# nicholasburden/pymarl

Hardware: AMD Instinct MI355X
Metric: learner samples/sec (B×T×n_agents), synthetic replay, 1/2/4/8 MI355X (higher is better)
Workload: dtype fp32; 1 GPU; QMIX synthetic replay n_agents=8 T=120 obs=80 state=168 batch=32; mixer=qmix, n_agents=8, n_actions=14, obs_dim=80, state_dim=168, episode_limit=120, batch_per_gpu=32, global_batch=32, replay_episodes=5000, parallelism=dp1

## Files before the change

include/mq_learner.h:

```cpp
#ifndef MQ_LEARNER_H
#define MQ_LEARNER_H

#include <stdint.h>

#ifdef __cplusplus
extern "C" {
#endif

enum { MQ_MIXER_NONE = 0, MQ_MIXER_VDN = 1, MQ_MIXER_QMIX = 2 };
enum { MQ_OK = 0, MQ_ERR_ARG = 1, MQ_ERR_HIP = 2, MQ_ERR_STATE = 3 };
enum { MQ_NSUMS = 8 };
enum { MQ_NSTATS = 8 };

enum {
  MQ_P_FC1_W, MQ_P_FC1_B, MQ_P_RNN_W_IH, MQ_P_RNN_W_HH, MQ_P_RNN_B_IH, MQ_P_RNN_B_HH, MQ_P_FC2_W, MQ_P_FC2_B,
  MQ_P_HW1_W, MQ_P_HW1_B, MQ_P_HWF_W, MQ_P_HWF_B, MQ_P_HB1_W, MQ_P_HB1_B, MQ_P_V0_W, MQ_P_V0_B, MQ_P_V2_W,
  MQ_P_V2_B, MQ_P_COUNT
};

typedef struct mq_config {
  int32_t n_agents, n_actions, obs_dim, state_dim;
  int32_t rnn_hidden_dim;
  int32_t mixing_embed_dim;
  int32_t mixer;
// ... 52 lines not shown
                   float* q_out, int32_t which, void* stream);
int mq_agent_forward(mq_handle* h, const float* inputs, int32_t rows, const float* h_in, float* h_out,
                     float* q_out, int32_t which, void* stream);
int mq_greedy_actions(const float* q, const int32_t* avail, int64_t* out, int32_t rows, int32_t n_actions,
                      void* stream);

int mq_qmix_forward(const float* mixer, int32_t n_agents, int32_t state_dim, int32_t embed_dim,
                    const float* agent_qs, const float* states, float* q_tot, int32_t rows, void* stream);

enum { MQ_HYP_NONE = 0, MQ_HYP_WS = 1, MQ_HYP_LDS = 2, MQ_HYP_GEMM = 3 };
enum { MQ_MIX_FAST16 = 0, MQ_MIX_FAST32 = 1, MQ_MIX_GENERIC = 2, MQ_MIX_STREAM = 3 };
typedef struct mq_plan {
  int32_t rows;
  int32_t fused_fwd;
  int32_t rw_fwd;
  int32_t fused_bwd;
  int32_t rw_bwd;
  int32_t inline_ids;
  int32_t hyper;
  int32_t mix;
  int32_t tiles;
  int32_t dwh;
  int32_t td_lambda;
} mq_plan;
int mq_last_plan(const mq_handle* h, mq_plan* out);

int mq_set_timing(mq_handle* h, int32_t slots, uint32_t phase_mask);
int mq_phase_times(mq_handle* h, float* ms, int32_t cap, int32_t* n);
const char* mq_phase_names(void);

#ifdef __cplusplus
}
#endif
#endif
```

pymarl_amd/_lib.py:

```python
from __future__ import annotations

import ctypes
import os

HERE = os.path.dirname(os.path.abspath(__file__))
LIB_PATH = os.environ.get("MQ_LEARNER_LIB", os.path.join(HERE, "lib", "libmq_learner.so"))

MIXER_NONE, MIXER_VDN, MIXER_QMIX = 0, 1, 2
NSUMS = 8
NSTATS = 8
PARAM_NAMES = [
    "fc1.weight", "fc1.bias", "rnn.weight_ih", "rnn.weight_hh", "rnn.bias_ih", "rnn.bias_hh", "fc2.weight",
    "fc2.bias", "hyper_w_1.weight", "hyper_w_1.bias", "hyper_w_final.weight", "hyper_w_final.bias",
    "hyper_b_1.weight", "hyper_b_1.bias", "V.0.weight", "V.0.bias", "V.2.weight", "V.2.bias",
]
P_COUNT = len(PARAM_NAMES)

EXPORTS = [
    "mq_last_error", "mq_create", "mq_destroy", "mq_param_offsets", "mq_bind", "mq_forward_backward", "mq_apply",
    "mq_train_step", "mq_update_targets", "mq_copy_intermediate", "mq_mac_forward", "mq_agent_forward",
    "mq_greedy_actions", "mq_set_timing", "mq_phase_times", "mq_phase_names", "mq_set_data_parallel",
    "mq_last_plan", "mq_qmix_forward",
    "mc_create", "mc_destroy", "mc_param_offsets", "mc_bind", "mc_train_step", "mc_update_targets", "mc_policy",
    "mc_copy_intermediate", "mc_set_timing", "mc_phase_times", "mc_last_critic_path", "mq_comm_unique_id", "mq_comm_attach",
# ... 26 lines not shown
class MQReplay(ctypes.Structure):
    _fields_ = [
        ("obs", ctypes.c_void_p), ("state", ctypes.c_void_p), ("actions", ctypes.c_void_p),
        ("avail_actions", ctypes.c_void_p), ("reward", ctypes.c_void_p), ("terminated", ctypes.c_void_p),
        ("filled", ctypes.c_void_p), ("ep_ids", ctypes.c_void_p), ("n_episodes", ctypes.c_int64),
        ("batch_size", ctypes.c_int32), ("t_len", ctypes.c_int32), ("t_stride", ctypes.c_int32),
        ("ep_ids_host", ctypes.c_void_p), ("avail_bits", ctypes.c_void_p),
    ]


class MCConfig(ctypes.Structure):
    _fields_ = [
        ("n_agents", ctypes.c_int32), ("n_actions", ctypes.c_int32), ("obs_dim", ctypes.c_int32),
        ("state_dim", ctypes.c_int32), ("rnn_hidden_dim", ctypes.c_int32), ("obs_last_action", ctypes.c_int32),
        ("obs_agent_id", ctypes.c_int32), ("mask_before_softmax", ctypes.c_int32), ("gamma", ctypes.c_float),
        ("td_lambda", ctypes.c_float), ("lr", ctypes.c_float), ("critic_lr", ctypes.c_float),
        ("optim_alpha", ctypes.c_float), ("optim_eps", ctypes.c_float), ("grad_norm_clip", ctypes.c_float),
        ("max_batch", ctypes.c_int32), ("max_seq", ctypes.c_int32),
    ]


class MQPlan(ctypes.Structure):
    _fields_ = [(k, ctypes.c_int32) for k in ("rows", "fused_fwd", "rw_fwd", "fused_bwd", "rw_bwd", "inline_ids",
                                               "hyper", "mix", "tiles", "dwh", "td_lambda")]

    def as_dict(self):
        return {k: int(getattr(self, k)) for k, _ in self._fields_}


HYP_NAMES = {0: "none", 1: "ws", 2: "lds", 3: "gemm"}
MIX_NAMES = {0: "fast16", 1: "fast32", 2: "generic", 3: "stream"}

INLINE_IDS = 256
COMM_ID_BYTES = 128


_LIB = None


class MQError(RuntimeError):
    pass


def load(required=True):
    global _LIB
    if _LIB is not None:
        return _LIB
# ... 134 lines not shown
```

pymarl_amd/csrc/gru_bwd_fused.hpp:

```cpp
#pragma once
#include <cstdlib>
#include "gru_fwd_fused.hpp"
#include "dwh_kernel.hpp"

namespace mq {

constexpr int BRP = 4 * H + 4;

struct alignas(16) BwdFusedLds {
  float gh[2][FCH][BRP];
  float gi[2][FCH][BRP];
  float x1[FCH][H + 4];
  float xin[FCH][FXP];
  float dx1[FCH][H + 4];
  float db1[4][H];
  float wih[G3][H + 1];
};

inline bool fused_bwd_ok(int I, int O, int A, int n, int64_t RT) { return fused_fwd_ok(I, O, A, n, RT); }

constexpr int BSTH = 16, BSTN = BSTH + 152;
template <int DWH = 0, bool STAMP = false>
__global__ __launch_bounds__(512) void gru_bwd_fused_kernel(Dims d, Rep rp, const float* __restrict__ P, Lay L,
                                                            Work w, int64_t slab_len, int64_t slab1_len) {
  __shared__ BwdFusedLds S;
  extern __shared__ float dyn[];
  __shared__ uint32_t bst[STAMP ? BSTN : 1];
  auto bstamp = [&](int slot) {
    if constexpr (STAMP) {
      uint64_t tt;
      __builtin_amdgcn_sched_barrier(0);
      asm volatile("s_memtime %0\n\ts_waitcnt lgkmcnt(0)" : "=s"(tt)::"memory");
      __builtin_amdgcn_sched_barrier(0);
      if ((threadIdx.x & 63) == 0) bst[slot] = (uint32_t)tt;
    }
  };
  if (threadIdx.x == 0) bstamp(0);
  if constexpr (DWH != 0) {
    static_assert(sizeof(BwdFusedLds) >= 2 * 4 * DWH_T * (DWH_T + 1) * sizeof(float), "dW_hyper tiles reuse the LDS");
    if ((int)blockIdx.x >= d.R) {
      const int half = (int)threadIdx.x >> 8;
      const int lin = min(2 * ((int)blockIdx.x - d.R) + half, w.dwh_n - 1);
      dwh_body<8, 4>(d, L, w.dHYP, w.S0, w.slab_mix, w.dwh_len, w.dwh_ns, w.dwh_tj, lin, (int)threadIdx.x & 255,
                        (float*)&S + half * 4 * DWH_T * (DWH_T + 1));
      return;
// ... 43 lines not shown
    const int b3 = (c16 >> 3) & 1, b2 = (c16 >> 2) & 1, u0 = 4 * (lt >> 4);
    f32x4 xr[12];
    {
      const float* Whh = P + L.o[MQ_P_RNN_W_HH];
#pragma unroll
      for (int kk = 0; kk < 12; ++kk) xr[kk] = *(const f32x4*)(Whh + (12 * c16 + kk) * H + u0);
    }
    auto k12_sum = [&](const f32x4 (&dv)[3]) {
      f32x2 aA = {0.0f, 0.0f}, aB = {0.0f, 0.0f};
#pragma unroll
      for (int m = 0; m < 3; ++m)
#pragma unroll
        for (int e = 0; e < 4; ++e) {
          const f32x2 dd = {dv[m][e], dv[m][e]};
          aA = pk_fma(wT[2 * (4 * m + e)], dd, aA);
          aB = pk_fma(wT[2 * (4 * m + e) + 1], dd, aB);
        }
      const float x = aA.x + row_ror8(aB.x), y = aA.y + row_ror8(aB.y);
      return quad_sum(x + row_half_mirror(y));
    };
    struct In { float g, aux, w2, wd, ci, ch, hq, gz; };
    const float* aux_base;
    int64_t aux_stride;
    if (q == 0) { aux_base = w.Hs + (int64_t)r * H + k - (int64_t)R * H; aux_stride = (int64_t)R * H; }
    else if (q == 3) { aux_base = (const float*)arow; aux_stride = 2 * (int64_t)d.n; }
    else { aux_base = w.dch + r; aux_stride = R; }
    const float* g_base = w.Gates + (int64_t)r * (4 * H) + q * H + k;
    const int e0 = q == 0 ? 1 : 0, e12 = (q == 1 || q == 2) ? 1 : 0;
    auto load = [&](int t, In& s) {
      const int tc = max(t, 0);
      const int idx = tc + (e0 & (tc == 0 ? 1 : 0)) - (e12 & (tc >= T ? 1 : 0));
      s.g = g_base[(int64_t)tc * R * (4 * H)];
      s.aux = aux_base[idx * aux_stride];
    };
    auto lookup_w2 = [&](In& s) { s.w2 = w2_s[__builtin_bit_cast(int, quad_bcast<3>(s.aux)) * H + k]; };
    const float m0 = q == 0 ? 1.0f : 0.0f, m1 = q == 1 ? 1.0f : 0.0f, m2 = q == 2 ? 1.0f : 0.0f;
    const float m3 = q == 3 ? 1.0f : 0.0f;
    float carry = 0.0f, db_i = 0.0f, db_h = 0.0f;
    auto coeffs = [&](int t, In& s) {
      const float gr = quad_bcast<0>(s.g), gz = quad_bcast<1>(s.g), gn = quad_bcast<2>(s.g), ghn = quad_bcast<3>(s.g);
      const float hp = t > 0 ? quad_bcast<0>(s.aux) : 0.0f;
      const float dchv = t < T ? quad_bcast<2>(s.aux) : 0.0f;
      const float an = (1.0f - gz) * (1.0f - gn * gn);
      const float ar = (an * ghn) * (gr * (1.0f - gr));
      const float az = (hp - gn) * (gz * (1.0f - gz));
      const float rzc = fmaf(m0, ar, m1 * az);
      s.ci = fmaf(m2 + m3, an, rzc);
      s.ch = fmaf(m2, an * gr, rzc);
      s.hq = m3 * hp;
      s.wd = dchv * s.w2;
      s.gz = gz;
    };
    auto lstep = [&](int t, const In& cur, In& nxt, In& ahead) {
      load(t - 3, ahead);
      const int p = t & (FCH - 1), cb = (t / FCH) & 1;
      const float dh = carry + cur.wd;
      const float mine_i = dh * cur.ci;
      const float mine_h = fmaf(dh, cur.ch, cur.hq);
      S.gh[cb][p][q * H + k] = mine_h;
      S.gi[cb][p][q * H + k] = mine_i;
      db_i = fmaf(1.0f - m3, mine_i, db_i);
      db_h = fmaf(1.0f - m3, mine_h, db_h);
      lds_barrier();
      const f32x4* d12 = (const f32x4*)(&S.gh[cb][p][12 * c16]);
      const f32x4 dv[3] = {d12[0], d12[1], d12[2]};
      lookup_w2(nxt);
      coeffs(t - 1, nxt);
      carry = fmaf(dh, cur.gz, k12_sum(dv));
      if constexpr (STAMP) { if (tid < 64 && Tp - 1 - t < BSTN - BSTH) bstamp(BSTH + Tp - 1 - t); }
    };
    In sa, sb, sc, sd;
    load(Tp - 1, sa);
    load(Tp - 2, sb);
    load(Tp - 3, sc);
    stage_common();
    {
      const int a0 = u0 + 2 * b3 + b2, a1 = u0 + 2 * b3 + 1 - b2;
      const int v0 = u0 + 2 * (1 - b3) + b2, v1 = u0 + 2 * (1 - b3) + 1 - b2;
      auto pick = [](const f32x4& x, int i) { return i == 0 ? x[0] : i == 1 ? x[1] : i == 2 ? x[2] : x[3]; };
      const int i0 = a0 - u0, i1 = a1 - u0, i2 = v0 - u0, i3 = v1 - u0;
#pragma unroll
      for (int kk = 0; kk < 12; ++kk) {
        wT[2 * kk] = f32x2{pick(xr[kk], i0), pick(xr[kk], i1)};
        wT[2 * kk + 1] = f32x2{pick(xr[kk], i2), pick(xr[kk], i3)};
      }
    }
    drain_vmem();
    lds_barrier();
    if (tid == 0) bstamp(1);
    lookup_w2(sa);
    coeffs(Tp - 1, sa);
    int t = Tp - 1;
    for (; t - 3 >= 0; t -= 4) {
      lstep(t, sa, sb, sd);
      lstep(t - 1, sb, sc, sa);
      lstep(t - 2, sc, sd, sb);
      lstep(t - 3, sd, sa, sc);
    }
    if (t >= 0) lstep(t, sa, sb, sd);
    if (t - 1 >= 0) lstep(t - 1, sb, sc, sa);
    if (t - 2 >= 0) lstep(t - 2, sc, sd, sb);
    if (tid == 0) bstamp(2);
    lds_barrier();
    lds_barrier();
    if (q < 3) { slab[o_bi + q * H + k] = db_i; slab[o_bh + q * H + k] = db_h; }
  } else {
    const int ptid = tid - 256, wv = ptid >> 6, lane = ptid & 63, g = lane >> 4, c16 = lane & 15;
    const int Kq = (I + 15) / 16 * 4;
    f32x4 acc_hh[3][4], acc_ih[3][4], acc_w1[7];
#pragma unroll
    for (int i = 0; i < 3; ++i)
#pragma unroll
      for (int jj = 0; jj < 4; ++jj) { acc_hh[i][jj] = f32x4{0, 0, 0, 0}; acc_ih[i][jj] = f32x4{0, 0, 0, 0}; }
#pragma unroll
    for (int i = 0; i < 7; ++i) acc_w1[i] = f32x4{0, 0, 0, 0};
    f32x4 dxa = {0, 0, 0, 0}, dxb = {0, 0, 0, 0};
    float db1p = 0.0f;

    constexpr int NX1 = FCH * H / 256, NXI = (FCH * 4 * FKQ + 255) / 256;
    float rx1[NX1], rxi[NXI];
    auto issue_rows = [&](int C) {
      const int t0 = FCH * C;
#pragma unroll
      for (int s = 0; s < NX1; ++s) {
// ... 72 lines not shown
          if (16 * nt >= 4 * Kq) break;
          acc_w1[nt] = mfma16x4(av, S.xin[row][16 * nt + c16], acc_w1[nt]);
        }
      }
    };
    float h_next = 0.0f, dch_n = 0.0f;
    int act_n = 0;
    auto fc2_fetch = [&](int t) {
      const int tc = max(t, 0);
      dch_n = w.dch[(int64_t)min(tc, T - 1) * R + r];
      act_n = *(const int*)(arow + (int64_t)tc * d.n);
    };
    auto fc2_grads = [&](int t) {
      const int p = t & (FCH - 1), cb = (t / FCH) & 1;
      const float dchv = t < T ? dch_n : 0.0f;
      const int a = act_n;
      fc2_fetch(t - 1);
      if (t < T && (a & 3) == q) {
        dw2_s[a * H + k] += dchv * h_next;
        if (k == 0) db2_s[a] += dchv;
      }
      h_next = S.gh[cb][p][3 * H + k];
    };
    fc2_fetch(Tp - 1);
    issue_rows(cl);
    stage_common();

    lds_barrier();
    for (int c = cl; c >= 0; --c) {
      const int C = c + 1;
      const bool work = C <= cl;
#pragma unroll
      for (int u = 0; u < FCH; ++u) {
        const int t = FCH * c + FCH - 1 - u;
        if (t >= Tp) continue;
        lds_barrier();
        fc2_grads(t);
        if (work) {
          if (u >= 1 && u <= 4) dw_rec(C, u - 1, u, false);
          if (u == 4) store_rows(C);
          if (u >= 5 && u <= 8) dw_rec(C, u - 5, u - 4, true);
          if (u >= 9 && u <= 12) dx1_part(C, 3 * (u - 9), 3 * (u - 8));
          if (u == 12) dx1_epi();
          if (u == 13) dw1_part(0, 1);
          if (u == 14) dw1_part(1, 2);
          if (u == 15) dw1_part(2, 4);
        }
        if (u == 5 && c < cl) issue_rows(c);
      }
    }
    auto write_rec = [&](const f32x4 (&acc)[3][4], int64_t o) {
#pragma unroll
      for (int i = 0; i < 3; ++i)
#pragma unroll
        for (int jj = 0; jj < 4; ++jj)
          *(f32x4*)&slab[o + (((3 * wv + i) * 4 + jj) * 64 + lane) * 4] = acc[i][jj];
    };
    dw_rec(0, 0, 4, false);
    if (ptid == 0) bstamp(6);
    store_rows(0);
    write_rec(acc_hh, o_hh);
    if (ptid == 0) bstamp(7);
    lds_barrier();
    if (ptid == 0) bstamp(8);
    dw_rec(0, 0, 4, true);
    if (ptid == 0) bstamp(9);
    write_rec(acc_ih, 0);
    if (ptid == 0) bstamp(10);
    dx1_part(0, 0, 12);
    dx1_epi();
    if (ptid == 0) bstamp(11);
    lds_barrier();
    dw1_part(0, 4);
    if (ptid == 0) bstamp(3);

    float* slab1 = w.slab_fc1 + (int64_t)blockIdx.x * slab1_len;
#pragma unroll
    for (int nt = 0; nt < 7; ++nt)
#pragma unroll
      for (int e = 0; e < 4; ++e) {
        const int m = 16 * wv + 4 * g + e, nn = 16 * nt + c16;
        if (nn < I) slab1[m * I + nn] = acc_w1[nt][e];
      }
    S.db1[g][16 * wv + c16] = db1p;
  }
  lds_barrier();
  if (tid == 0) bstamp(4);
  for (int i = tid; i < A * H; i += 512) slab[o_w2 + i] = dw2_s[i];
  for (int i = tid; i < A; i += 512) slab[o_b2 + i] = db2_s[i];
  if (tid < H)
    w.slab_fc1[(int64_t)blockIdx.x * slab1_len + H * I + tid] =
        (S.db1[0][tid] + S.db1[1][tid]) + (S.db1[2][tid] + S.db1[3][tid]);
  if constexpr (STAMP) {
    asm volatile("s_waitcnt vmcnt(0)" ::: "memory");
    __syncthreads();
    if (tid == 0) bstamp(5);
    __syncthreads();
    if (blockIdx.x < 8)
      for (int i = tid; i < BSTN; i += 512) ((uint32_t*)w.GI)[(size_t)blockIdx.x * BSTN + i] = bst[i];
  }
}

inline void launch_bwd_fused_dwh(size_t dyn, hipStream_t s, const Dims& d, const Rep& rp, const float* P,
                                 const Lay& L, const Work& w, int64_t slab_len, int64_t slab1_len) {
  const dim3 grid(d.R + (w.dwh_n + 1) / 2);
  hipLaunchKernelGGL((gru_bwd_fused_kernel<1>), grid, dim3(512), dyn, s, d, rp, P, L, w, slab_len, slab1_len);
}
inline void launch_bwd_fused(dim3 grid, size_t dyn, hipStream_t s, const Dims& d, const Rep& rp, const float* P,
                             const Lay& L, const Work& w, int64_t slab_len, int64_t slab1_len, bool stamp = false) {
  if (stamp)
    hipLaunchKernelGGL((gru_bwd_fused_kernel<0, true>), grid, dim3(512), dyn, s, d, rp, P, L, w, slab_len, slab1_len);
  else
    hipLaunchKernelGGL((gru_bwd_fused_kernel<0>), grid, dim3(512), dyn, s, d, rp, P, L, w, slab_len, slab1_len);
}

}
```

pymarl_amd/csrc/gru_fwd_pair.hpp:

```cpp
#pragma once
#include "gru_fwd_fused.hpp"

namespace mq {

struct alignas(16) PairLds {
  float h0[H];
  int psync[4];
  float xin[2][FCH][FXP];
  float x1[2][2][FCH][H + 4];
  float hs[2][2][FCH][H + 4];
  float gi[2][2][FCH][G3];
  f32x4 grec[2][FCH][H];
};
static_assert(sizeof(PairLds) - offsetof(PairLds, hs) >= 2 * G3 * H * sizeof(float), "W_hh staging fits");
constexpr int kPairPrologueBarriers = 3;

inline bool pair_fwd_ok(int I, int O, int A, int n, int64_t RT) { return fused_fwd_ok(I, O, A, n, RT); }

constexpr int PSH = 32;
constexpr int PST = PSH + 2 * 512;
MQ_DEV uint32_t stamp_now() {
  uint64_t t;
  __builtin_amdgcn_sched_barrier(0);
  asm volatile("s_memtime %0\n\ts_waitcnt lgkmcnt(0)" : "=s"(t)::"memory");
// ... 379 lines not shown
      for (int e = 0; e < 4; ++e) S.gi[z][cc & 1][4 * g + e][16 * (3 * pw + s) + c16] = accg[s][e] + bih[z][s];
  };
  auto fc2 = [&](int cc) {
    const int z = pw;
    f32x4 q0 = {0, 0, 0, 0}, q1 = {0, 0, 0, 0};
#pragma unroll
    for (int kq = 0; kq < 4; ++kq) {
      const f32x4 av = *(const f32x4*)&S.hs[z][cc & 1][c16][16 * g + 4 * kq];
      q0 = mfma16x4(av[0], w2r[4 * kq], q0);
      q1 = mfma16x4(av[1], w2r[4 * kq + 1], q1);
      q0 = mfma16x4(av[2], w2r[4 * kq + 2], q0);
      q1 = mfma16x4(av[3], w2r[4 * kq + 3], q1);
    }
    const int t0 = FCH * cc;
    const auto qb = buf_rsrc(w.Q + (int64_t)z * d.RT() * A + ((int64_t)t0 * R + r) * A);
    const uint32_t lo = (uint32_t)(4 * g) * RA + c16;
#pragma unroll
    for (int e = 0; e < 4; ++e)
      buf_st(qb, (t0 + 4 * g + e < Tp && c16 < A) ? (lo + e * RA) * 4 : kDrop, (q0[e] + q1[e]) + b2);
  };

  auto store_records = [&](int cc) {
    const int t0 = FCH * cc, j = ptid & 63;
#pragma unroll
    for (int k = 0; k < 4; ++k) {
      const int i = 4 * k + (ptid >> 6), t = t0 + i;
      const f32x4 gv = S.grec[cc & 1][i][j];
      const float hv = S.hs[0][cc & 1][i][j];
      const bool ok = t < Tp;
      buf_st(buf_rsrc(w.Hs + (int64_t)min(t, Tp - 1) * RH), ok ? ((uint32_t)r * H + j) * 4 : kDrop, hv);
      const auto gb = buf_rsrc(w.Gates + (int64_t)min(t, Tp - 1) * (4 * RH));
      const uint32_t go = ((uint32_t)r * (4 * H) + j) * 4;
#pragma unroll
      for (int q = 0; q < 4; ++q) buf_st(gb, ok ? go + q * 4 * H : kDrop, gv[q]);
    }
  };

  if (pw == 0) stamp(16);
  store_gather(0);
  if (cl >= 1) issue_gather(1);
  if (pw == 0) stamp(17);
  lds_barrier();
  if (pw == 0) stamp(18);
  fc1(0, 0);
  fc1(1, 0);
  if (cl >= 1) { store_gather(1); if (cl >= 2) issue_gather(2); }
// ... 90 lines not shown
```

pymarl_amd/csrc/learner_types.hpp:

```cpp
#pragma once
#include "common.hpp"
#include "../../include/mq_learner.h"

namespace mq {

constexpr int H = 64;
constexpr int G3 = 3 * H;

struct Dims {
  int n, A, O, S, E, I, NH;
  int B, Tp, T, R, M;
  int t_stride;
  int last_action, agent_id, mixer, double_q;
  float gamma;
  float huber;
  FastDiv dR, dN, dB, dO, dI, dS;
  MQ_DEV int64_t RT() const { return (int64_t)Tp * R; }
};

MQ_DEV float td_loss(float mtd, float delta) {
  if (delta > 0.0f) {
    const float ax = fabsf(mtd);
    return ax <= delta ? 0.5f * mtd * mtd : delta * (ax - 0.5f * delta);
  }
// ... 26 lines not shown
  float* X1;
  float* GI;
  float* Hs;
  float* Gates;
  float* Q;
  float* HYP;
  float* dHYP;
  float* dch;
  float* dGI;
  float* dP1;
  float* slab_fc1;
  float* slab_rnn;
  float* slab_mix;
  float* slab_v2;
  float* loss_part;
  float* norm_part;
  int32_t* curmax;
  float* red_tmp;
  float* XIN;
  float* S0;
  float* dHo;
  int64_t dwh_len = 0;
  int dwh_ns = 0, dwh_tj = 0, dwh_n = 0;
};

MQ_DEV void split_tr(const Dims& d, uint32_t tr, int& t, int& r, int& b, int& ag) {
  t = (int)fdiv(tr, d.dR);
  r = (int)tr - t * d.R;
  b = (int)fdiv((uint32_t)r, d.dN);
  ag = r - b * d.n;
}

}
```

pymarl_amd/csrc/mq_learner.hip:

```cpp
#include <cstdio>
#include <cstdlib>
#include <algorithm>
#include <cstring>
#include <mutex>
#include <string>
#include <vector>

#include <rccl/rccl.h>
#include "learner_gemms.hpp"
#include "gru_kernels.hpp"
#include "gru_fwd_fused.hpp"
#include "gru_fwd_pair.hpp"
#include "gru_bwd_fused.hpp"
#include "gru_tiles.hpp"
#include "mix_kernels.hpp"
#include "td_lambda_kernel.hpp"
#include "hyper_kernel.hpp"
#include "dwh_kernel.hpp"
#include "optim_kernels.hpp"
#include "module_fwd.hpp"
#include "switches.hpp"

using namespace mq;

// ... 76 lines not shown
  float *on = nullptr, *tg = nullptr, *grad = nullptr, *sq = nullptr, *stats = nullptr;
  int32_t* curmax_user = nullptr;
  void* ws = nullptr;
  Work w;
  int32_t* curmax_ws = nullptr;
  bool have_fb = false;
  Dims last;
  mq_plan plan{};
  int nsplit_fc1 = 1, nsplit_mix = 1, nblk_bwd = 1, nblk_mix = 1, n_norm_part = 0;
  bool force_unfused = plan_flag("unfused_fwd");
  bool force_unfused_bwd = plan_flag("unfused_bwd");
  static constexpr int fused_bwd_rmax = 512;
  int dwh_split = plan_int("dwh_split", 8);
  int row_tiles = plan_int("row_tiles", -1);
  bool dp = false;
  ncclComm_t comm = nullptr;
  int comm_world = 0;
  bool comm_owned = false;
  hipStream_t side = nullptr;
  hipEvent_t ev_fork = nullptr, ev_join = nullptr;
  int hyp_in_fwd = plan_int("hyp_in_fwd", -1);
  int dwh_in_bwd = plan_int("dwh_in_bwd", -1);
  int fwd_pair = plan_int("fwd_pair", -1);
  bool pair_hyp_epi = plan_flag("pair_hyp_epi");
  bool mix_generic = plan_flag("mix_generic");
  bool lambda_path = plan_int("lambda_path", 0) != 0;
  float *YT = nullptr, *G = nullptr;
  bool have_lambda = false;
  int num_cu = 0;
  int slots = 0;
  uint32_t mask = 0;
  int64_t tstep = 0;
  std::vector<hipEvent_t> ev0, ev1;
  std::vector<uint8_t> ev_used;
};

namespace {

void compute_layout(mq_handle* h) {
  const mq_config& c = h->cfg;
  const int Hd = mq::H, n = c.n_agents, A = c.n_actions, S = c.state_dim, E = h->E, I = h->I;
  int64_t sz[MQ_P_COUNT] = {};
  sz[MQ_P_FC1_W] = (int64_t)Hd * I; sz[MQ_P_FC1_B] = Hd;
  sz[MQ_P_RNN_W_IH] = 3LL * Hd * Hd; sz[MQ_P_RNN_W_HH] = 3LL * Hd * Hd;
  sz[MQ_P_RNN_B_IH] = 3 * Hd; sz[MQ_P_RNN_B_HH] = 3 * Hd;
  sz[MQ_P_FC2_W] = (int64_t)A * Hd; sz[MQ_P_FC2_B] = A;
// ... 225 lines not shown
  mq_handle* h = new mq_handle();
  h->cfg = c;
  h->E = c.mixer == MQ_MIXER_QMIX ? c.mixing_embed_dim : 0;
  h->I = c.obs_dim + (c.obs_last_action ? c.n_actions : 0) + (c.obs_agent_id ? c.n_agents : 0);
  h->NH = h->E * (c.n_agents + 3);
  compute_layout(h);

  const int64_t n = c.n_agents, A = c.n_actions, Hd = mq::H;
  const int64_t RT = (int64_t)c.max_seq * c.max_batch * n;
  const int64_t Mm = (int64_t)(c.max_seq - 1) * c.max_batch;
  const int64_t Rm = (int64_t)c.max_batch * n;
  const int64_t nmix = (Mm + 3) / 4;
  const int64_t NH = h->NH;
  auto ng = [](int64_t ns) { return std::min<int64_t>(ns, kRedZ); };
  const int64_t nfc1 = std::max<int64_t>(kNsplitMax, Rm);
  const int64_t red_tmp = ng(Rm) * h->len_rnn + ng(nfc1) * (Hd * h->I + Hd) + ng(kNsplitMax) * h->len_mix +
                          ng(nmix) * (h->E + 1) + ng(nmix) * 8;
  const int64_t norm_parts = (Hd * h->I + Hd + 255) / 256 + (h->len_rnn + 255) / 256 + (h->len_mix + 255) / 256 +
                             (h->E + 1 + 255) / 256 + 1 + 8;
  int64_t sizes[20] = {
      2 * RT * Hd,
      2 * RT * 3 * Hd,
      2 * RT * Hd,
      RT * 4 * Hd,
      2 * RT * A,
      2 * Mm * NH,
      Mm * NH,
      Mm * n,
      RT * 3 * Hd,
      RT * Hd,
      nfc1 * (Hd * h->I + Hd),
      Rm * h->pitch_rnn,
      (int64_t)kNsplitMax * h->len_mix,
      nmix * (h->E + 1),
      nmix * 8,
      std::max<int64_t>(norm_parts, 256),
      Mm * n,
      red_tmp,
      RT * h->I,
      Mm * c.state_dim,
  };
  int64_t total = 0, offs[20];
  for (int i = 0; i < 20; ++i) { offs[i] = total; total += align_up(std::max<int64_t>(sizes[i], 1)); }
  hipError_t e = hipMalloc(&h->ws, total * sizeof(float));
  if (e != hipSuccess) {
    delete h;
    return set_err(MQ_ERR_HIP, std::string("workspace hipMalloc(") + std::to_string(total * 4) + " B): " +
// ... 71 lines not shown
    return set_err(MQ_ERR_STATE, "training needs online, target, grad, sq_avg and stats bound (mq_bind)");
  int rc = check_batch(h, batch);
  if (rc) return rc;
  const Dims d = make_dims(h, batch);
  const Rep rp = make_rep(batch);
  const Lay L = make_lay(h);
  Work w = h->w;
  int32_t* curmax = h->curmax_user ? h->curmax_user : h->curmax_ws;
  const int64_t RT = (int64_t)d.Tp * d.R;
  PhaseTimer pt{h, s};
  const mq_config& c = h->cfg;

  mq_plan plan{};
  plan.rows = d.R;
  plan.inline_ids = rp.nids > 0 ? 1 : 0;
  const int rw_bwd = std::min(2, pick_rw(d.R, 256));
  const int kq1 = tile_kq1(d.O);
  const bool tiles = tiles_ok(d.I, d.O, d.A, d.n, d.Tp, RT) && !h->force_unfused && !h->force_unfused_bwd &&
                     (h->row_tiles == 1 || (h->row_tiles < 0 && d.R > 512));
  const bool fused_bwd = !tiles && d.R <= h->fused_bwd_rmax && fused_bwd_ok(d.I, d.O, d.A, d.n, RT) &&
                         !h->force_unfused_bwd;
  const int rw_fwd = pick_rw(d.R, 512);
  bool hyp_in_fwd = false;
  plan.tiles = tiles ? 1 : 0;
  if (tiles) {
    pt.begin(PH_GRUF);
    const dim3 grid(16 * (((d.R + TR_F - 1) / TR_F + 7) / 8));
    const float *P0 = h->on, *P1 = h->tg;
    if (kq1 == 8) hipLaunchKernelGGL(gru_fwd_tile_kernel<8>, grid, dim3(512), 0, s, d, rp, P0, P1, L, w);
    else if (kq1 == 20) hipLaunchKernelGGL(gru_fwd_tile_kernel<20>, grid, dim3(512), 0, s, d, rp, P0, P1, L, w);
    else if (kq1 == 40) hipLaunchKernelGGL(gru_fwd_tile_kernel<40>, grid, dim3(512), 0, s, d, rp, P0, P1, L, w);
    else if (kq1 == 72) hipLaunchKernelGGL(gru_fwd_tile_kernel<72>, grid, dim3(512), 0, s, d, rp, P0, P1, L, w);
    else hipLaunchKernelGGL(gru_fwd_tile_kernel<80>, grid, dim3(512), 0, s, d, rp, P0, P1, L, w);
    MQ_HIP(hipGetLastError());
  } else if (rw_fwd == 1 && fused_fwd_ok(d.I, d.O, d.A, d.n, RT) && !h->force_unfused) {
    plan.fused_fwd = 1;
    pt.begin(PH_GRUF);
    const bool two_waves = device_cus(h) > 0 && d.R > h->num_cu;
    const bool pair = h->hyp_in_fwd != 1 && pair_fwd_ok(d.I, d.O, d.A, d.n, RT) &&
                      (h->fwd_pair == 1 || (h->fwd_pair < 0 && !two_waves && device_cus(h) > 0));
    hyp_in_fwd = !pair && (h->hyp_in_fwd == 1 || (h->hyp_in_fwd < 0 && two_waves)) && c.mixer == MQ_MIXER_QMIX &&
                 hyper_ws_ok(d.S, d.E, d.NH, d.M) && hyf_ok(d.S, d.E, d.NH, d.M);
    if (hyp_in_fwd) {
      plan.hyper = MQ_HYP_WS;
      launch_fwd_fused_hyp(s, d, rp, (const float*)h->on, (const float*)h->tg, L, w);
    } else if (pair) {
      plan.fused_fwd = 2;
      hyp_in_fwd = h->hyp_in_fwd != 0 && c.mixer == MQ_MIXER_QMIX && hyper_ws_ok(d.S, d.E, d.NH, d.M) &&
                   hyf_ok(d.S, d.E, d.NH, d.M);
      if (hyp_in_fwd) plan.hyper = MQ_HYP_WS;
      std::string stamp_path;
      const bool want_stamp = env_item("MQ_DIAG", "pair_stamp", &stamp_path) && !stamp_path.empty();
      const int hsched = env_int("MQ_DIAG", "hyp_sched", kHypSched, 16);
      const int pair_hyp = !hyp_in_fwd ? 0 : (2 * ((d.M + 31) / 32) <= d.R && !h->pair_hyp_epi) ? 2 : 1;
      const bool stamp = want_stamp && d.Tp <= 512 && FCH * d.O <= 256 * 5;
      launch_fwd_pair(s, d, rp, (const float*)h->on, (const float*)h->tg, L, w, pair_hyp, stamp, hsched);
      if (stamp) {
        std::vector<uint32_t> st((size_t)8 * PST);
        MQ_HIP(hipMemcpyAsync(st.data(), w.slab_rnn, st.size() * 4, hipMemcpyDeviceToHost, s));
        MQ_HIP(hipStreamSynchronize(s));
        if (FILE* f = fopen(stamp_path.c_str(), "ab")) { fwrite(st.data(), 4, st.size(), f); fclose(f); }
      }
    } else {
      launch_fwd_fused(dim3(d.R, 2), s, d, rp, (const float*)h->on, (const float*)h->tg, L, w);
    }
    MQ_HIP(hipGetLastError());
  } else {
    plan.rw_fwd = rw_fwd;
    pt.begin(PH_FC1);
    {
      Fc1Prob p{d, rp, h->on, h->tg, h->off[MQ_P_FC1_W], h->off[MQ_P_FC1_B], w.X1, w.XIN, RT};
      MQ_HIP(launch_gemm(p, (int)RT, 2 * mq::H, 1, s));
    }
    pt.begin(PH_GI);
    {
      GiProb p{w.X1, h->on, h->tg, h->off[MQ_P_RNN_W_IH], h->off[MQ_P_RNN_B_IH], w.GI, RT};
      MQ_HIP(launch_gemm(p, (int)RT, mq::G3, 2, s));
    }
// ... 83 lines not shown
  } else if (fused_bwd) {
    const bool many = device_cus(h) > 0 && d.R > h->num_cu;
    h->nblk_bwd = d.R;
    h->nsplit_fc1 = h->nblk_bwd;
    const size_t dyn = ((size_t)2 * d.A * mq::H + d.A) * sizeof(float);
    if (c.mixer == MQ_MIXER_QMIX) {
      const int tj = (d.NH + DWH_T - 1) / DWH_T, ts = (d.S + 1 + DWH_T - 1) / DWH_T;
      dwh_mode = h->dwh_in_bwd >= 0 ? (h->dwh_in_bwd ? 1 : 0) : many ? 1 : 0;
      if (dwh_mode != 0) {
        w.dwh_tj = tj;
        w.dwh_ns = dwh_ns;
        w.dwh_n = tj * ts * dwh_ns;
        w.dwh_len = h->len_mix;
        h->nsplit_mix = dwh_ns;
      }
    }
    dwh_in_bwd = dwh_mode != 0;
    plan.dwh = dwh_mode;
    const float* P0 = (const float*)h->on;
    const int64_t l1 = (int64_t)mq::H * d.I + mq::H;
    std::string bstamp_path;
    const bool bstamp = dwh_mode != 1 && env_item("MQ_DIAG", "bwd_stamp", &bstamp_path) && !bstamp_path.empty() &&
                        d.Tp <= BSTN - BSTH;
    if (dwh_mode == 1) MQ_LDS(gru_bwd_fused_kernel<1>, dyn);
    else MQ_LDS((gru_bwd_fused_kernel<0, true>), dyn);
    if (dwh_mode == 1) launch_bwd_fused_dwh(dyn, s, d, rp, P0, L, w, h->pitch_rnn, l1);
    else launch_bwd_fused(dim3(d.R), dyn, s, d, rp, P0, L, w, h->pitch_rnn, l1, bstamp);
    if (bstamp) {
      std::vector<uint32_t> st((size_t)8 * BSTN);
      MQ_HIP(hipMemcpyAsync(st.data(), w.GI, st.size() * 4, hipMemcpyDeviceToHost, s));
      MQ_HIP(hipStreamSynchronize(s));
      if (FILE* f = fopen(bstamp_path.c_str(), "ab")) { fwrite(st.data(), 4, st.size(), f); fclose(f); }
    }
    MQ_HIP(hipGetLastError());
  } else {
    {
      const size_t dyn = ((size_t)2 * d.A * mq::H + d.A) * sizeof(float);
      if (rw_bwd == 1) MQ_LDS(gru_bwd_kernel<1>, dyn);
      else if (rw_bwd == 2) MQ_LDS(gru_bwd_kernel<2>, dyn);
      else MQ_LDS(gru_bwd_kernel<4>, dyn);
      hipError_t e = rw_bwd == 1 ? launch_gru_bwd<1>(d, rp, h, L, w, s, &h->nblk_bwd)
                   : rw_bwd == 2 ? launch_gru_bwd<2>(d, rp, h, L, w, s, &h->nblk_bwd)
                                 : launch_gru_bwd<4>(d, rp, h, L, w, s, &h->nblk_bwd);
      MQ_HIP(e);
    }
    pt.begin(PH_DX1);
    {
      Dx1Prob p{w.dGI, h->on + h->off[MQ_P_RNN_W_IH], w.X1, w.dP1, RT};
      MQ_HIP(launch_gemm(p, (int)RT, mq::H, 1, s));
    }
// ... 304 lines not shown
```

Before: 154.7 million samples/s.

## Add lean fused GRU backward with precomputed gate coefficients and walked addressing

Adds a lean variant of the fused GRU backward kernel, on by default when the paired forward path runs. The forward pair kernel now stores precomputed GRU derivative coefficients (ar, az, an, anr, gz) into a widened 5H gate record. The backward loads these instead of recomputing them on its serial time recurrence, and walks pointers for addressing instead of computing per-step indices. The fc2 gradient accumulation becomes register-resident packed FMAs fed from lane-broadcast prefetches. In exchange the Gates buffer grows by a quarter, and the forward does extra stores and arithmetic.

```diff
diff --git a/include/mq_learner.h b/include/mq_learner.h
--- a/include/mq_learner.h
+++ b/include/mq_learner.h
@@ -98,6 +98,7 @@
   int32_t tiles;
   int32_t dwh;
   int32_t td_lambda;
+  int32_t bwd_lean;
 } mq_plan;
 int mq_last_plan(const mq_handle* h, mq_plan* out);
 
diff --git a/pymarl_amd/_lib.py b/pymarl_amd/_lib.py
--- a/pymarl_amd/_lib.py
+++ b/pymarl_amd/_lib.py
@@ -72,7 +72,7 @@
 
 class MQPlan(ctypes.Structure):
     _fields_ = [(k, ctypes.c_int32) for k in ("rows", "fused_fwd", "rw_fwd", "fused_bwd", "rw_bwd", "inline_ids",
-                                               "hyper", "mix", "tiles", "dwh", "td_lambda")]
+                                               "hyper", "mix", "tiles", "dwh", "td_lambda", "bwd_lean")]
 
     def as_dict(self):
         return {k: int(getattr(self, k)) for k, _ in self._fields_}
diff --git a/pymarl_amd/csrc/gru_bwd_fused.hpp b/pymarl_amd/csrc/gru_bwd_fused.hpp
--- a/pymarl_amd/csrc/gru_bwd_fused.hpp
+++ b/pymarl_amd/csrc/gru_bwd_fused.hpp
@@ -1,5 +1,6 @@
 #pragma once
 #include <cstdlib>
+#include <type_traits>
 #include "gru_fwd_fused.hpp"
 #include "dwh_kernel.hpp"
 
@@ -19,8 +20,10 @@
 
 inline bool fused_bwd_ok(int I, int O, int A, int n, int64_t RT) { return fused_fwd_ok(I, O, A, n, RT); }
 
+constexpr int LEAN_ADDR = 1, LEAN_FC2 = 2, LEAN_COEF = 4;
+constexpr int kBwdLean = LEAN_ADDR | LEAN_FC2 | LEAN_COEF;
 constexpr int BSTH = 16, BSTN = BSTH + 152;
-template <int DWH = 0, bool STAMP = false>
+template <int DWH = 0, bool STAMP = false, int LEAN = 0>
 __global__ __launch_bounds__(512) void gru_bwd_fused_kernel(Dims d, Rep rp, const float* __restrict__ P, Lay L,
                                                             Work w, int64_t slab_len, int64_t slab1_len) {
   __shared__ BwdFusedLds S;
@@ -110,37 +113,56 @@
     struct In { float g, aux, w2, wd, ci, ch, hq, gz; };
     const float* aux_base;
     int64_t aux_stride;
+    constexpr bool COEF = (LEAN & LEAN_COEF) != 0;
+    constexpr int GP = COEF ? 5 * H : 4 * H;
     if (q == 0) { aux_base = w.Hs + (int64_t)r * H + k - (int64_t)R * H; aux_stride = (int64_t)R * H; }
     else if (q == 3) { aux_base = (const float*)arow; aux_stride = 2 * (int64_t)d.n; }
+    else if (COEF && q == 1) { aux_base = w.Gates + (int64_t)r * GP + 4 * H + k; aux_stride = (int64_t)R * GP; }
     else { aux_base = w.dch + r; aux_stride = R; }
-    const float* g_base = w.Gates + (int64_t)r * (4 * H) + q * H + k;
-    const int e0 = q == 0 ? 1 : 0, e12 = (q == 1 || q == 2) ? 1 : 0;
+    const float* g_base = w.Gates + (int64_t)r * GP + q * H + k;
+    const int e0 = q == 0 ? 1 : 0, e12 = ((q == 1 && !COEF) || q == 2) ? 1 : 0;
     auto load = [&](int t, In& s) {
       const int tc = max(t, 0);
       const int idx = tc + (e0 & (tc == 0 ? 1 : 0)) - (e12 & (tc >= T ? 1 : 0));
-      s.g = g_base[(int64_t)tc * R * (4 * H)];
+      s.g = g_base[(int64_t)tc * R * GP];
       s.aux = aux_base[idx * aux_stride];
+    };
+    const float* g_walk = w.Gates + (int64_t)(Tp - 4) * R * GP;
+    const uint32_t g_lane = (uint32_t)r * GP + q * H + k;
+    const char* aux_walk = (const char*)(aux_base + (int64_t)(Tp - 4) * aux_stride);
+    const uint32_t aux_step = (uint32_t)aux_stride * 4;
+    auto load_walk = [&](In& s) {
+      s.g = ld_u32(g_walk, g_lane);
+      s.aux = *(const float*)aux_walk;
+      g_walk -= (int64_t)R * GP;
+      aux_walk -= aux_step;
     };
     auto lookup_w2 = [&](In& s) { s.w2 = w2_s[__builtin_bit_cast(int, quad_bcast<3>(s.aux)) * H + k]; };
     const float m0 = q == 0 ? 1.0f : 0.0f, m1 = q == 1 ? 1.0f : 0.0f, m2 = q == 2 ? 1.0f : 0.0f;
     const float m3 = q == 3 ? 1.0f : 0.0f;
     float carry = 0.0f, db_i = 0.0f, db_h = 0.0f;
-    auto coeffs = [&](int t, In& s) {
-      const float gr = quad_bcast<0>(s.g), gz = quad_bcast<1>(s.g), gn = quad_bcast<2>(s.g), ghn = quad_bcast<3>(s.g);
+    auto coeffs = [&](auto fuse, int t, In& s) {
       const float hp = t > 0 ? quad_bcast<0>(s.aux) : 0.0f;
       const float dchv = t < T ? quad_bcast<2>(s.aux) : 0.0f;
-      const float an = (1.0f - gz) * (1.0f - gn * gn);
-      const float ar = (an * ghn) * (gr * (1.0f - gr));
-      const float az = (hp - gn) * (gz * (1.0f - gz));
-      const float rzc = fmaf(m0, ar, m1 * az);
-      s.ci = fmaf(m2 + m3, an, rzc);
-      s.ch = fmaf(m2, an * gr, rzc);
+      if constexpr (COEF) {
+        s.ci = s.g;
+        s.ch = fmaf(m2, quad_bcast<3>(s.g), (m0 + m1) * s.g);
+        s.gz = quad_bcast<1>(s.aux);
+      } else {
+        const float gr = quad_bcast<0>(s.g), gz = quad_bcast<1>(s.g), gn = quad_bcast<2>(s.g);
+        const float ghn = quad_bcast<3>(s.g);
+        const GruCoef c = gru_coef(gr, gz, gn, ghn, hp, decltype(fuse)::value);
+        const float rzc = fmaf(m0, c.ar, m1 * c.az);
+        s.ci = fmaf(m2 + m3, c.an, rzc);
+        s.ch = fmaf(m2, c.anr, rzc);
+        s.gz = gz;
+      }
       s.hq = m3 * hp;
       s.wd = dchv * s.w2;
-      s.gz = gz;
-    };
-    auto lstep = [&](int t, const In& cur, In& nxt, In& ahead) {
-      load(t - 3, ahead);
+    };
+    auto lstep = [&](auto walk, auto fuse, int t, const In& cur, In& nxt, In& ahead) {
+      if constexpr (decltype(walk)::value) load_walk(ahead);
+      else load(t - 3, ahead);
       const int p = t & (FCH - 1), cb = (t / FCH) & 1;
       const float dh = carry + cur.wd;
       const float mine_i = dh * cur.ci;
@@ -153,7 +175,7 @@
       const f32x4* d12 = (const f32x4*)(&S.gh[cb][p][12 * c16]);
       const f32x4 dv[3] = {d12[0], d12[1], d12[2]};
       lookup_w2(nxt);
-      coeffs(t - 1, nxt);
+      coeffs(fuse, t - 1, nxt);
       carry = fmaf(dh, cur.gz, k12_sum(dv));
       if constexpr (STAMP) { if (tid < 64 && Tp - 1 - t < BSTN - BSTH) bstamp(BSTH + Tp - 1 - t); }
     };
@@ -177,17 +199,29 @@
     lds_barrier();
     if (tid == 0) bstamp(1);
     lookup_w2(sa);
-    coeffs(Tp - 1, sa);
+    coeffs(std::true_type{}, Tp - 1, sa);
     int t = Tp - 1;
+    constexpr std::false_type by_t{};
+    constexpr std::true_type fu{};
+    constexpr std::false_type unf{};
+    if constexpr ((LEAN & LEAN_ADDR) != 0) {
+      constexpr std::true_type walk{};
+      for (; t - 6 >= 1; t -= 4) {
+        lstep(walk, fu, t, sa, sb, sd);
+        lstep(walk, fu, t - 1, sb, sc, sa);
+        lstep(walk, unf, t - 2, sc, sd, sb);
+        lstep(walk, fu, t - 3, sd, sa, sc);
+      }
+    }
     for (; t - 3 >= 0; t -= 4) {
-      lstep(t, sa, sb, sd);
-      lstep(t - 1, sb, sc, sa);
-      lstep(t - 2, sc, sd, sb);
-      lstep(t - 3, sd, sa, sc);
-    }
-    if (t >= 0) lstep(t, sa, sb, sd);
-    if (t - 1 >= 0) lstep(t - 1, sb, sc, sa);
-    if (t - 2 >= 0) lstep(t - 2, sc, sd, sb);
+      lstep(by_t, fu, t, sa, sb, sd);
+      lstep(by_t, fu, t - 1, sb, sc, sa);
+      lstep(by_t, unf, t - 2, sc, sd, sb);
+      lstep(by_t, fu, t - 3, sd, sa, sc);
+    }
+    if (t >= 0) lstep(by_t, fu, t, sa, sb, sd);
+    if (t - 1 >= 0) lstep(by_t, fu, t - 1, sb, sc, sa);
+    if (t - 2 >= 0) lstep(by_t, fu, t - 2, sc, sd, sb);
     if (tid == 0) bstamp(2);
     lds_barrier();
     lds_barrier();
@@ -306,7 +340,33 @@
       }
       h_next = S.gh[cb][p][3 * H + k];
     };
-    fc2_fetch(Tp - 1);
+    float fin_c = 0.0f, fin_n = 0.0f;
+    f32x2 acc2[4] = {{0.0f, 0.0f}, {0.0f, 0.0f}, {0.0f, 0.0f}, {0.0f, 0.0f}};
+    auto issue_fc2 = [&](int C, float& fin) {
+      const int tt = FCH * C + (lane & 15);
+      const float* src = (lane & 16) ? (const float*)(arow + (int64_t)min(tt, Tp - 1) * d.n)
+                                     : w.dch + (int64_t)max(min(tt, T - 1), 0) * R + r;
+      fin = *src;
+    };
+    auto fc2_lean = [&](int t, int p) {
+      const int cb = (t / FCH) & 1;
+      const float dchv = t < T ? __builtin_bit_cast(float, __builtin_amdgcn_readlane(__builtin_bit_cast(int, fin_c), p))
+                               : 0.0f;
+      const int amq = __builtin_amdgcn_readlane(__builtin_bit_cast(int, fin_c), 16 + p) - q;
+      const f32x2 h1 = {h_next, 1.0f};
+#pragma unroll
+      for (int j = 0; j < 4; ++j) {
+        const float m = amq == 4 * j ? dchv : 0.0f;
+        acc2[j] = pk_fma(f32x2{m, m}, h1, acc2[j]);
+      }
+      h_next = S.gh[cb][p][3 * H + k];
+    };
+    if constexpr ((LEAN & LEAN_FC2) != 0) {
+      issue_fc2(cl, fin_c);
+      if (cl >= 1) issue_fc2(cl - 1, fin_n);
+    } else {
+      fc2_fetch(Tp - 1);
+    }
     issue_rows(cl);
     stage_common();
 
@@ -314,12 +374,14 @@
     for (int c = cl; c >= 0; --c) {
       const int C = c + 1;
       const bool work = C <= cl;
+      if constexpr ((LEAN & LEAN_FC2) != 0) { if (c < cl) fin_c = fin_n; }
 #pragma unroll
       for (int u = 0; u < FCH; ++u) {
         const int t = FCH * c + FCH - 1 - u;
         if (t >= Tp) continue;
         lds_barrier();
-        fc2_grads(t);
+        if constexpr ((LEAN & LEAN_FC2) != 0) fc2_lean(t, FCH - 1 - u);
+        else fc2_grads(t);
         if (work) {
           if (u >= 1 && u <= 4) dw_rec(C, u - 1, u, false);
           if (u == 4) store_rows(C);
@@ -330,6 +392,7 @@
           if (u == 14) dw1_part(1, 2);
           if (u == 15) dw1_part(2, 4);
         }
+        if constexpr ((LEAN & LEAN_FC2) != 0) { if (u == 5 && c < cl && c >= 1) issue_fc2(c - 1, fin_n); }
         if (u == 5 && c < cl) issue_rows(c);
       }
     }
@@ -367,6 +430,16 @@
         if (nn < I) slab1[m * I + nn] = acc_w1[nt][e];
       }
     S.db1[g][16 * wv + c16] = db1p;
+    if constexpr ((LEAN & LEAN_FC2) != 0) {
+#pragma unroll
+      for (int j = 0; j < 4; ++j) {
+        const int a = 4 * j + q;
+        if (a < A) {
+          dw2_s[a * H + k] = acc2[j].x;
+          if (k == 0) db2_s[a] = acc2[j].y;
+        }
+      }
+    }
   }
   lds_barrier();
   if (tid == 0) bstamp(4);
@@ -385,17 +458,25 @@
   }
 }
 
+#define MQ_BWD_FUSED_LAUNCH(DW, ST, LN) \
+  hipLaunchKernelGGL((gru_bwd_fused_kernel<DW, ST, LN>), grid, dim3(512), dyn, s, d, rp, P, L, w, slab_len, slab1_len)
 inline void launch_bwd_fused_dwh(size_t dyn, hipStream_t s, const Dims& d, const Rep& rp, const float* P,
-                                 const Lay& L, const Work& w, int64_t slab_len, int64_t slab1_len) {
+                                 const Lay& L, const Work& w, int64_t slab_len, int64_t slab1_len, bool lean) {
   const dim3 grid(d.R + (w.dwh_n + 1) / 2);
-  hipLaunchKernelGGL((gru_bwd_fused_kernel<1>), grid, dim3(512), dyn, s, d, rp, P, L, w, slab_len, slab1_len);
+  if (lean) MQ_BWD_FUSED_LAUNCH(1, false, kBwdLean);
+  else MQ_BWD_FUSED_LAUNCH(1, false, 0);
 }
 inline void launch_bwd_fused(dim3 grid, size_t dyn, hipStream_t s, const Dims& d, const Rep& rp, const float* P,
-                             const Lay& L, const Work& w, int64_t slab_len, int64_t slab1_len, bool stamp = false) {
-  if (stamp)
-    hipLaunchKernelGGL((gru_bwd_fused_kernel<0, true>), grid, dim3(512), dyn, s, d, rp, P, L, w, slab_len, slab1_len);
-  else
-    hipLaunchKernelGGL((gru_bwd_fused_kernel<0>), grid, dim3(512), dyn, s, d, rp, P, L, w, slab_len, slab1_len);
+                             const Lay& L, const Work& w, int64_t slab_len, int64_t slab1_len, bool lean,
+                             bool stamp = false) {
+  if (stamp) {
+    if (lean) MQ_BWD_FUSED_LAUNCH(0, true, kBwdLean);
+    else MQ_BWD_FUSED_LAUNCH(0, true, 0);
+  } else {
+    if (lean) MQ_BWD_FUSED_LAUNCH(0, false, kBwdLean);
+    else MQ_BWD_FUSED_LAUNCH(0, false, 0);
+  }
 }
+#undef MQ_BWD_FUSED_LAUNCH
 
 }
diff --git a/pymarl_amd/csrc/gru_fwd_pair.hpp b/pymarl_amd/csrc/gru_fwd_pair.hpp
--- a/pymarl_amd/csrc/gru_fwd_pair.hpp
+++ b/pymarl_amd/csrc/gru_fwd_pair.hpp
@@ -425,6 +425,25 @@
 
   auto store_records = [&](int cc) {
     const int t0 = FCH * cc, j = ptid & 63;
+    if (w.rec_coef) {
+#pragma unroll 1
+      for (int k = 0; k < 4; ++k) {
+        const int i = 4 * k + (ptid >> 6), t = t0 + i;
+        const f32x4 gv = S.grec[cc & 1][i][j];
+        const float hv = S.hs[0][cc & 1][i][j];
+        const float hp = *(i > 0 ? &S.hs[0][cc & 1][i - 1][j] : &S.h0[j]);
+        const bool ok = t < Tp;
+        buf_st(buf_rsrc(w.Hs + (int64_t)min(t, Tp - 1) * RH), ok ? ((uint32_t)r * H + j) * 4 : kDrop, hv);
+        const GruCoef cf = gru_coef(gv[0], gv[1], gv[2], gv[3], hp, coef_fused(t, Tp));
+        const auto gb = buf_rsrc(w.Gates + (int64_t)min(t, Tp - 1) * (5 * RH));
+        const uint32_t go = ((uint32_t)r * (5 * H) + j) * 4;
+        const float pl[5] = {cf.ar, cf.az, cf.an, cf.anr, gv[1]};
+#pragma unroll
+        for (int q = 0; q < 5; ++q) buf_st(gb, ok ? go + q * 4 * H : kDrop, pl[q]);
+      }
+      if (ptid < H) S.h0[j] = S.hs[0][cc & 1][FCH - 1][j];
+      return;
+    }
 #pragma unroll
     for (int k = 0; k < 4; ++k) {
       const int i = 4 * k + (ptid >> 6), t = t0 + i;
diff --git a/pymarl_amd/csrc/learner_types.hpp b/pymarl_amd/csrc/learner_types.hpp
--- a/pymarl_amd/csrc/learner_types.hpp
+++ b/pymarl_amd/csrc/learner_types.hpp
@@ -72,7 +72,21 @@
   float* dHo;
   int64_t dwh_len = 0;
   int dwh_ns = 0, dwh_tj = 0, dwh_n = 0;
+  int rec_coef = 0;
 };
+
+MQ_DEV bool coef_fused(int t, int Tp) { return t > Tp - 4 || ((Tp - t) & 3) != 0; }
+struct GruCoef { float ar, az, an, anr; };
+MQ_DEV GruCoef gru_coef(float gr, float gz, float gn, float ghn, float hp, bool fuse_n2) {
+#pragma clang fp contract(off)
+  GruCoef c;
+  const float n2 = gn * gn;
+  c.an = (1.0f - gz) * (fuse_n2 ? fmaf(-gn, gn, 1.0f) : 1.0f - n2);
+  c.ar = (c.an * ghn) * (gr * (1.0f - gr));
+  c.az = (hp - gn) * (gz * (1.0f - gz));
+  c.anr = c.an * gr;
+  return c;
+}
 
 MQ_DEV void split_tr(const Dims& d, uint32_t tr, int& t, int& r, int& b, int& ag) {
   t = (int)fdiv(tr, d.dR);
diff --git a/pymarl_amd/csrc/mq_learner.hip b/pymarl_amd/csrc/mq_learner.hip
--- a/pymarl_amd/csrc/mq_learner.hip
+++ b/pymarl_amd/csrc/mq_learner.hip
@@ -122,6 +122,7 @@
   int hyp_in_fwd = plan_int("hyp_in_fwd", -1);
   int dwh_in_bwd = plan_int("dwh_in_bwd", -1);
   int fwd_pair = plan_int("fwd_pair", -1);
+  int bwd_lean = plan_int("bwd_lean", -1);
   bool pair_hyp_epi = plan_flag("pair_hyp_epi");
   bool mix_generic = plan_flag("mix_generic");
   bool lambda_path = plan_int("lambda_path", 0) != 0;
@@ -393,7 +394,7 @@
       2 * RT * Hd,
       2 * RT * 3 * Hd,
       2 * RT * Hd,
-      RT * 4 * Hd,
+      RT * 5 * Hd,
       2 * RT * A,
       2 * Mm * NH,
       Mm * NH,
@@ -511,6 +512,7 @@
                          !h->force_unfused_bwd;
   const int rw_fwd = pick_rw(d.R, 512);
   bool hyp_in_fwd = false;
+  bool pair_fwd = false;
   plan.tiles = tiles ? 1 : 0;
   if (tiles) {
     pt.begin(PH_GRUF);
@@ -535,6 +537,7 @@
       launch_fwd_fused_hyp(s, d, rp, (const float*)h->on, (const float*)h->tg, L, w);
     } else if (pair) {
       plan.fused_fwd = 2;
+      pair_fwd = true;
       hyp_in_fwd = h->hyp_in_fwd != 0 && c.mixer == MQ_MIXER_QMIX && hyper_ws_ok(d.S, d.E, d.NH, d.M) &&
                    hyf_ok(d.S, d.E, d.NH, d.M);
       if (hyp_in_fwd) plan.hyper = MQ_HYP_WS;
@@ -543,6 +546,7 @@
       const int hsched = env_int("MQ_DIAG", "hyp_sched", kHypSched, 16);
       const int pair_hyp = !hyp_in_fwd ? 0 : (2 * ((d.M + 31) / 32) <= d.R && !h->pair_hyp_epi) ? 2 : 1;
       const bool stamp = want_stamp && d.Tp <= 512 && FCH * d.O <= 256 * 5;
+      w.rec_coef = fused_bwd && h->bwd_lean != 0 && (kBwdLean & LEAN_COEF) != 0 ? 1 : 0;
       launch_fwd_pair(s, d, rp, (const float*)h->on, (const float*)h->tg, L, w, pair_hyp, stamp, hsched);
       if (stamp) {
         std::vector<uint32_t> st((size_t)8 * PST);
@@ -672,10 +676,17 @@
     std::string bstamp_path;
     const bool bstamp = dwh_mode != 1 && env_item("MQ_DIAG", "bwd_stamp", &bstamp_path) && !bstamp_path.empty() &&
                         d.Tp <= BSTN - BSTH;
-    if (dwh_mode == 1) MQ_LDS(gru_bwd_fused_kernel<1>, dyn);
-    else MQ_LDS((gru_bwd_fused_kernel<0, true>), dyn);
-    if (dwh_mode == 1) launch_bwd_fused_dwh(dyn, s, d, rp, P0, L, w, h->pitch_rnn, l1);
-    else launch_bwd_fused(dim3(d.R), dyn, s, d, rp, P0, L, w, h->pitch_rnn, l1, bstamp);
+    const bool lean = pair_fwd && h->bwd_lean != 0;
+    plan.bwd_lean = lean ? 1 : 0;
+    if (lean) {
+      if (dwh_mode == 1) MQ_LDS((gru_bwd_fused_kernel<1, false, kBwdLean>), dyn);
+      else MQ_LDS((gru_bwd_fused_kernel<0, true, kBwdLean>), dyn);
+    } else {
+      if (dwh_mode == 1) MQ_LDS(gru_bwd_fused_kernel<1>, dyn);
+      else MQ_LDS((gru_bwd_fused_kernel<0, true>), dyn);
+    }
+    if (dwh_mode == 1) launch_bwd_fused_dwh(dyn, s, d, rp, P0, L, w, h->pitch_rnn, l1, lean);
+    else launch_bwd_fused(dim3(d.R), dyn, s, d, rp, P0, L, w, h->pitch_rnn, l1, lean, bstamp);
     if (bstamp) {
       std::vector<uint32_t> st((size_t)8 * BSTN);
       MQ_HIP(hipMemcpyAsync(st.data(), w.GI, st.size() * 4, hipMemcpyDeviceToHost, s));
```

Result: faster. 161.8 million samples/s, median of 6 (+4.6%).
